# driskai/scenario_gym

Measured on AMD Instinct MI355X. Metric: entity-steps/sec (batched rollout), higher is better.
Workload: dtype f64

## Files before the change

scenario_gym_amd/csrc/sgym_control.hpp:

```cpp
#pragma once

namespace sg {

struct CtlLds { double ctrl[9][64]; double seg[5][64]; };

template <bool FAST, bool RIDERS = false>
__device__ __forceinline__ void control_body_l(CtlLds &lds ,
                                               const unsigned qblock ,
                                               const Params &p, double timestep, int n_steps, int first, int k0,
                                               const double *actions , double *tab, int row0, int metrics)
{
    const int lane = threadIdx.x;
    const size_t q = (size_t)qblock * 64 + lane;
    const int ent_raw = p.ctl_ent[q];
    const bool active = ent_raw >= 0;
    const uint32_t ent = active ? (uint32_t)ent_raw : 0u;
    const uint32_t r = ent / (uint32_t)p.EP;
    const LanePtr st(p.stat + (size_t)(ent >> 6) * (ST_COUNT * 64), (ent & 63) * 8u);
    const LanePtr dy(p.dyn + (size_t)(ent >> 6) * ((size_t)p.FROWS * 64), (ent & 63) * 8u);
    const int64_t meta = fld<int64_t>(st, ST_META);
    const int kind = active ? (int)(meta & 0xff) : SG_KIND_NONE;
    const double min_t = fld(st, ST_MIN_T), bl = fld(st, ST_BL);
    const bool is_ego = active && (int)(ent - r * (uint32_t)p.EP) == p.sstat[r].ego;
#pragma unroll
    for (int c = 0; c < 9; ++c) lds.ctrl[c][lane] = fld(st, ST_CTRL + c);
    const size_t NP = (size_t)p.n_ctl_pad;
    double *cst = p.ctl_state + q;

    double pose[6], t, prev_t;
    double m_avg, m_max, m_t;
    bool present;
    CtrlState cs;
    if (first) {
        const sg_scenario_state &sd = p.sdyn[r];
        t = sd.t;
        prev_t = sd.prev_t;
        m_avg = sd.ego_avg_speed; m_max = sd.ego_max_speed; m_t = sd.avg_t;
        present = fld<uint64_t>(dy, SG_F_PRESENT) != 0;
#pragma unroll
        for (int c = 0; c < 6; ++c) pose[c] = fld(dy, SG_F_POSE + c);
        cs.speed = fld(dy, SG_F_CTRL + 0); cs.e_lon_prev = fld(dy, SG_F_CTRL + 1);
        cs.e_lat_prev = fld(dy, SG_F_CTRL + 2); cs.e_lon_int = fld(dy, SG_F_CTRL + 3);
    } else {
#pragma unroll
        for (int c = 0; c < 6; ++c) pose[c] = cst[(CS_POSE + c) * NP];
        present = cst[CS_PRESENT * NP] != 0.0;
        cs.speed = cst[(CS_CTRL + 0) * NP]; cs.e_lon_prev = cst[(CS_CTRL + 1) * NP];
        cs.e_lat_prev = cst[(CS_CTRL + 2) * NP]; cs.e_lon_int = cst[(CS_CTRL + 3) * NP];
        t = cst[CS_T * NP];
        prev_t = cst[CS_PREV_T * NP];
        m_avg = cst[(CS_METRIC + 0) * NP]; m_max = cst[(CS_METRIC + 1) * NP]; m_t = cst[(CS_METRIC + 2) * NP];
    }
    if (!active) present = false;

    Table T;
    {
        const double *kn = p.knots + fld<int64_t>(st, ST_KNOT_OFF) * 7;
        T.x = kn; T.xs = 7; T.y = kn + 1; T.ys = 7; T.cs = 1;
        T.n = active ? (int)(meta >> 32) : 0;
    }
    double seg_hi;
    int seg_cur;
    double sgr[5] = {0.0, 0.0, 0.0, 0.0, 0.0};
    auto seg_publish = [&](const Segment &S) {
        lds.seg[0][lane] = S.x_lo;
        lds.seg[1][lane] = S.ylo[0]; lds.seg[2][lane] = S.ylo[1];
        lds.seg[3][lane] = S.sl[0]; lds.seg[4][lane] = S.sl[1];
        if (FAST) { sgr[0] = S.x_lo; sgr[1] = S.ylo[0]; sgr[2] = S.ylo[1]; sgr[3] = S.sl[0]; sgr[4] = S.sl[1]; }
        seg_hi = S.x_hi;
        seg_cur = S.cur;
    };
    {
        Segment S;
        S.cur = seg_locate(T, t);
        seg_load(T, S);
        seg_publish(S);
    }
    double *out = tab + (q * (size_t)(p.tab_steps + 1) + (size_t)row0) * CT_W;
    double *out1 = out + (size_t)p.n_ctl_pad * ((size_t)(p.tab_steps + 1) * CT_W);
    double *out2 = out1 + (size_t)p.n_ctl_pad * ((size_t)(p.tab_steps + 1) * CT_W);
    const bool replay_lane = RIDERS && (kind == SG_KIND_REPLAY || kind == SG_KIND_AGENT_REPLAY);
    const double max_t = fld(st, ST_MAX_T);
    const bool is_static = (int)(meta >> 32) == 1;
    Table TR{};
    Segment SR{};
    if (RIDERS) {
        TR = lane_table(p, replay_lane ? kind : SG_KIND_NONE, p.sstat[r], (int)(ent - r * (uint32_t)p.EP), st);
        if (!replay_lane) TR.n = 0;
        SR.cur = seg_locate(TR, t);
        seg_load(TR, SR);
    }
    sg_loads_done();
    const bool fast_kind = FAST && !p.ctl_general && sg_all(!active || (kind == SG_KIND_AGENT_PID && bl > 0.0 && bl < 0x1p400));
    const RecipDiv rd_l(active ? bl : 1.0), rd_10(10.0);
    double cpr[9];
#pragma unroll
    for (int c = 0; c < 9; ++c) cpr[c] = FAST ? fld(st, ST_CTRL + c) : 0.0;
    sg_loads_done();

    for (int k = 0; k < n_steps; ++k) {
        const double *Kp = SG_TRIG;
        if (!FAST) asm volatile("" : "+s"(Kp));
        ConstTbl K = (ConstTbl)Kp;
        const double next_t = t + timestep;
        const double state_dt = t - prev_t;
        const double dt = next_t - t;
        if (FAST && fast_kind && sg_all(!active || (present && !(next_t > seg_hi) && __builtin_fabs(pose[3]) < 1.0e5))) {
            const double dq = next_t - sgr[0];
            const double tx = sgr[3] * dq + sgr[1], ty = sgr[4] * dq + sgr[2];
            double sin_h, cos_h;
            sg_sincos_core(pose[3], sin_h, cos_h, K);
            const double e0 = tx - pose[0], e1 = ty - pose[1];
            const double e_lon = cos_h * e0 + sin_h * e1;
            const double e_lat = -sin_h * e0 + cos_h * e1;
            const double speed0 = cs.speed;
            const double g_mid = 1.0 - rd_10.div(0.9 * (speed0 - 5.0));
            const double gain = (speed0 > 5.0 && speed0 <= 15) ? g_mid : (speed0 > 15 ? 0.1 : 1.0);
            const RecipDiv rd(state_dt);
            const double d_lat = e_lat - cs.e_lat_prev, d_lon = e_lon - cs.e_lon_prev;
            const double e_lat_D = rd.div(d_lat);
            const double kp = cpr[SG_C_STEER_KP] * gain, kd = cpr[SG_C_STEER_KD] * gain;
            double steer = kp * e_lat + kd * e_lat_D;
            const double e_lon_D = rd.div(d_lon);
            const double e_lon_I = cs.e_lon_int + e_lon * state_dt;
            double accel = cpr[SG_C_ACCEL_KP] * e_lon + cpr[SG_C_ACCEL_KD] * e_lon_D + cpr[SG_C_ACCEL_KI] * e_lon_I;
            accel = __builtin_fabs(e_lon) > 0.1 ? accel : 0.0;
            const double max_steer = cpr[SG_C_MAX_STEER], max_accel = cpr[SG_C_MAX_ACCEL];
            const double max_speed = cpr[SG_C_MAX_SPEED], allow_rev = cpr[SG_C_ALLOW_REVERSE];
            accel = __builtin_fmin(__builtin_fmax(accel, -max_accel), max_accel);
            steer = __builtin_fmin(__builtin_fmax(steer, -max_steer), max_steer);
            const double dxs = speed0 * cos_h, dys = speed0 * sin_h;
            double tan_s = sg_tan_poly(steer, K);
            const bool steep = !(__builtin_fabs(steer) < 0.67434);
            if (sg_any(steep & active)) {
                double s2, c2;
                sg_sincos_core(steer, s2, c2, K);
                tan_s = steep ? s2 / c2 : tan_s;
            }
            const double hnum = speed0 * tan_s;
            const double dh = hnum == 0.0 ? hnum : rd_l.div(hnum);
            const double nx = pose[0] + dxs * dt, ny = pose[1] + dys * dt, nh = pose[3] + dh * dt;
            double nspeed = speed0 + accel * dt;
            nspeed = allow_rev == 0.0 ? __builtin_fmax(0.0, nspeed) : nspeed;
            nspeed = max_speed == max_speed ? __builtin_fmin(max_speed, nspeed) : nspeed;
            bool ok = rd.safe(d_lat) & rd.safe(d_lon) & (__builtin_fabs(steer) < 1.0e5) & (rd_l.safe(hnum) | (hnum == 0.0));
            double n_avg = m_avg, n_max = m_max, n_mt = m_t;
            if (metrics) {
                const RecipDiv rdt(dt), rnt(next_t);
                const double ax = nx - pose[0], ay = ny - pose[1];
                const double az = pose[2] - pose[2];
                const double speed = sg_norm3(rdt.div(ax), rdt.div(ay), 0.0);
                const double w = rnt.div(m_t);
                n_avg = m_avg + (1.0 - w) * (speed - m_avg);
                n_max = __builtin_fmax(speed, m_max);
                n_mt = next_t;
                ok = ok & (!is_ego | (rdt.safe(ax) & rdt.safe(ay) & rnt.safe(m_t) & (dt > 0.0) & (az == 0.0)));
            }
            if (sg_all(!active || ok)) {
                cs.e_lat_prev = e_lat; cs.e_lon_prev = e_lon; cs.e_lon_int = e_lon_I; cs.speed = nspeed;
                pose[0] = nx; pose[1] = ny; pose[3] = nh;
                if (is_ego) { m_avg = n_avg; m_max = n_max; m_t = n_mt; }
                prev_t = t;
                t = next_t;
                *reinterpret_cast<double4 *>(out + (size_t)k * CT_W) = make_double4(pose[0], pose[1], pose[3], cs.speed);
                *reinterpret_cast<double4 *>(out1 + (size_t)k * CT_W) = make_double4(cs.e_lon_prev, cs.e_lat_prev, cs.e_lon_int, 0.0);
                if (is_ego && metrics) *reinterpret_cast<double4 *>(out2 + (size_t)k * CT_W) = make_double4(m_avg, m_max, m_t, 0.0);
                continue;
            }
        }
        double act_a = 0.0, act_s = 0.0;
        if (kind == SG_KIND_AGENT_VEHICLE && actions) {
            const double *a = actions + ((size_t)(k0 + k) * p.R + r) * 2;
            act_a = a[0];
            act_s = a[1];
        }
        if (next_t > seg_hi) {
            Segment S;
            S.x_hi = seg_hi;
            S.cur = seg_cur;
            seg_advance(T, S, next_t);
            seg_publish(S);
            sg_loads_done();
        }
        double np_[6];
        const double dq = next_t - lds.seg[0][lane];
        np_[0] = lds.seg[3][lane] * dq + lds.seg[1][lane];
        np_[1] = lds.seg[4][lane] * dq + lds.seg[2][lane];
        bool npres = false;
        if (RIDERS && replay_lane) {
            if (next_t > SR.x_hi) { seg_advance(TR, SR, next_t); sg_loads_done(); }
            const double dqr = next_t - SR.x_lo;
#pragma unroll
            for (int c = 0; c < 6; ++c) np_[c] = SR.sl[c] * dqr + SR.ylo[c];
            npres = kind == SG_KIND_REPLAY ? (p.persist || is_static || (next_t >= min_t && next_t <= max_t))
                                           : (present || min_t >= t);
        } else if (present) {
            npres = true;
            const double tx = np_[0], ty = np_[1];
#pragma unroll
            for (int c = 0; c < 6; ++c) np_[c] = pose[c];
            double sin_h, cos_h;
            sg_sincos(pose[3], sin_h, cos_h, K);
            auto cp = [&](int q) -> double { return lds.ctrl[q][lane]; };
            if (kind == SG_KIND_AGENT_PID)
                pid_step(cs, cp, bl, state_dt, dt, tx, ty, sin_h, cos_h, np_, K);
            else
                vehicle_step(cs, cp, bl, dt, act_a, act_s, sin_h, cos_h, np_, K);
        } else if (active && min_t >= t) {
            npres = true;
            Segment S;
            S.cur = seg_cur;
            seg_load(T, S);
            sg_loads_done();
            const double dqs = next_t - S.x_lo;
#pragma unroll
            for (int c = 0; c < 6; ++c) np_[c] = S.sl[c] * dqs + S.ylo[c];
        }
        if (is_ego && npres && metrics) {
            double prev[6];
            if (!present) {
                own_position_extrap(T.x, T.n, t, prev);
                sg_loads_done();
            } else {
#pragma unroll
                for (int c = 0; c < 6; ++c) prev[c] = pose[c];
            }
            const double v0 = (np_[0] - prev[0]) / dt, v1 = (np_[1] - prev[1]) / dt, v2 = (np_[2] - prev[2]) / dt;
            const double speed = sg_norm3(v0, v1, v2);
            const double w = m_t / next_t;
            m_avg += (1.0 - w) * (speed - m_avg);
            m_t = next_t;
            m_max = __builtin_fmax(speed, m_max);
        }
        present = npres;
        if (npres) {
#pragma unroll
            for (int c = 0; c < 6; ++c) pose[c] = np_[c];
        }
        prev_t = t;
        t = next_t;
        *reinterpret_cast<double4 *>(out + (size_t)k * CT_W) = make_double4(pose[0], pose[1], pose[3], cs.speed);
        *reinterpret_cast<double4 *>(out1 + (size_t)k * CT_W) = make_double4(cs.e_lon_prev, cs.e_lat_prev, cs.e_lon_int, 0.0);
        if (is_ego && metrics) *reinterpret_cast<double4 *>(out2 + (size_t)k * CT_W) = make_double4(m_avg, m_max, m_t, 0.0);
        if (RIDERS) *reinterpret_cast<double4 *>(out2 + (size_t)k * CT_W) = make_double4(pose[2], pose[4], pose[5], present ? 1.0 : 0.0);
    }
#pragma unroll
    for (int c = 0; c < 6; ++c) cst[(CS_POSE + c) * NP] = pose[c];
    cst[CS_PRESENT * NP] = present ? 1.0 : 0.0;
    cst[(CS_CTRL + 0) * NP] = cs.speed; cst[(CS_CTRL + 1) * NP] = cs.e_lon_prev;
    cst[(CS_CTRL + 2) * NP] = cs.e_lat_prev; cst[(CS_CTRL + 3) * NP] = cs.e_lon_int;
    cst[CS_T * NP] = t;
    cst[CS_PREV_T * NP] = prev_t;
    cst[(CS_METRIC + 0) * NP] = m_avg; cst[(CS_METRIC + 1) * NP] = m_max; cst[(CS_METRIC + 2) * NP] = m_t;
}

template <bool FAST, bool RIDERS = false>
__device__ __forceinline__ void control_body(const Params &p, double timestep, int n_steps, int first, int k0,
                                             const double *actions , double *tab, int row0, int metrics)
{
    __shared__ CtlLds lds;
    control_body_l<FAST, RIDERS>(lds, blockIdx.x, p, timestep, n_steps, first, k0, actions, tab, row0, metrics);
}

#ifdef SG_UNIT_CTL
static __global__ __launch_bounds__(64, SG_CTL_WAVES) void control_kernel(Params p, double timestep, int n_steps, int first, int k0,
                                                     const double *actions , double *tab, int row0, int metrics)
{
    control_body<false>(p, timestep, n_steps, first, k0, actions, tab, row0, metrics);
}
#endif
#ifdef SG_UNIT_CTL
static __global__ __launch_bounds__(64, 2) void control_kernel_riders(Params p, double timestep, int n_steps, int first, int k0,
                                                               const double *actions , double *tab, int row0, int metrics)
{
    control_body<false, true>(p, timestep, n_steps, first, k0, actions, tab, row0, 0);
}
#endif
#ifdef SG_UNIT_CTL
static __global__ __launch_bounds__(64, 1) void control_kernel_fast(Params p, double timestep, int n_steps, int first, int k0,
                                                             const double *actions , double *tab, int row0, int metrics)
{
#ifdef SG_CTL_SETPRIO
    __builtin_amdgcn_s_setprio(3);
#endif
    control_body<true>(p, timestep, n_steps, first, k0, actions, tab, row0, metrics);
}
#endif

}
```

scenario_gym_amd/csrc/sgym_core.hpp:

```cpp
#pragma once

namespace sg {

enum {
    ST_BW = 0, ST_BL, ST_BCX, ST_BCY,
    ST_MIN_T, ST_MAX_T,
    ST_KNOT_OFF,
    ST_META,
    ST_ROUTE,
    ST_CTL,
    ST_CTRL,
    NCTRL_ROWS = 13,
    ST_COUNT = ST_CTRL + NCTRL_ROWS
};
constexpr uint32_t ROW = 512;

struct ScenStatic {
    double t0, length;
    int64_t grid_off;
    int32_t grid_n, ego;
};

struct RoadNet { double x0, y0, inv_cell; int32_t nx, ny; int64_t cell_base; };
struct RoadCand { int32_t poly; uint32_t edge_off; uint16_t n_edges; uint8_t ref_sel, ref_inside; };
// ... 48 lines not shown
    int ctl_general;
    int ped_serial;
    int quiet;
    int tab_steps;
    int noise_mode;
    double noise_std_lon, noise_std_lat;
    const double *noise_normals;
    long long noise_len;
    unsigned long long noise_seed;
    int ped_behaviour;
    int n_ped_models;
    const double *ped_models;
    const int32_t *model_of;
#ifdef SG_PHASE_TIMERS
    unsigned long long *phase_cycles;
#endif
};

enum { PM_BEHAVIOUR = 0, PM_SF = 1, PM_STD_LON = 13, PM_STD_LAT = 14, PM_W = 16 };
static_assert(sizeof(sg_social_force) == 12 * sizeof(double), "sg_social_force is twelve doubles");

enum { CT_X = 0, CT_Y, CT_H, CT_SPEED, CT_W = 4, CT_ELON = 0, CT_ELAT, CT_EINT, CT_MAVG = 0, CT_MMAX, CT_MT, CT_PLANES = 3 };
enum { CS_POSE = 0, CS_PRESENT = 6, CS_CTRL = 7, CS_T = 11, CS_PREV_T = 12, CS_METRIC = 13, CS_COUNT = 16 };

#define SG_GLOBAL __attribute__((address_space(1)))
struct LanePtr {
    SG_GLOBAL char *a[3];
    __device__ __forceinline__ LanePtr(const double *blk, uint32_t voff)
    {
        a[0] = (SG_GLOBAL char *)(reinterpret_cast<char *>(const_cast<double *>(blk)) + voff);
        a[1] = a[0] + 8 * ROW;
        a[2] = a[0] + 16 * ROW;
        asm("" : "+v"(a[1]), "+v"(a[2]));
    }
};
template <typename T = double>
__device__ __forceinline__ T fld(const LanePtr &lp, int f)
{
    const int b = f < 24 ? f >> 3 : 2;
    return *reinterpret_cast<SG_GLOBAL const T *>(lp.a[b] + (f - 8 * b) * (int)ROW);
}
template <typename T>
__device__ __forceinline__ void stf(const LanePtr &lp, int f, T v)
{
    const int b = f < 24 ? f >> 3 : 2;
    *reinterpret_cast<SG_GLOBAL T *>(lp.a[b] + (f - 8 * b) * (int)ROW) = v;
}

__device__ __forceinline__ double sg_norm3(double a, double b, double c)
{
    return __builtin_sqrt(__builtin_fma(c, c, __builtin_fma(b, b, a * a)));
}
__device__ __forceinline__ double sg_norm2(double a, double b)
{
    return __builtin_sqrt(__builtin_fma(b, b, a * a));
}

__device__ __noinline__ double2 sg_sincos_slow(double x)
{
    return make_double2(sin(x), cos(x));
}

static __constant__ double SG_TRIG[48] = {
    6.36619772367581382433e-01,
    1.57079632673412561417e+00,
    6.07710050630396597660e-11,
    2.02226624879595063154e-21,
    -1.66666666666666324348e-01, 8.33333333332248946124e-03, -1.98412698298579493134e-04,
    2.75573137070700676789e-06, -2.50507602534068634195e-08, 1.58969099521155010221e-10,
    4.16666666666666019037e-02, -1.38888888888741095749e-03, 2.48015872894767294178e-05,
    -2.75573143513906633035e-07, 2.08757232129817482790e-09, -1.13596475577881948265e-11,
    3.33333333333334091986e-01, 1.33333333333201242699e-01, 5.39682539762260521377e-02,
    2.18694882948595424599e-02, 8.86323982359930005737e-03, 3.59207910759131235356e-03,
    1.45620945432529025516e-03, 5.88041240820264096874e-04, 2.46463134818469906812e-04,
    7.81794442939557092300e-05, 7.14072491382608190305e-05, -1.85586374855275456654e-05,
    2.59073051863633712884e-05, 0.0, 0.0, 0.0,
    3.33333333333329318027e-01, -1.99999999998764832476e-01, 1.42857142725034663711e-01, -1.11111104054623557880e-01,
    9.09088713343650656196e-02, -7.69187620504482999495e-02, 6.66107313738753120669e-02, -5.83357013379057348645e-02,
    4.97687799461593236017e-02, -3.65315727442169155270e-02, 1.62858201153657823623e-02, 0.0, 0.0, 0.0, 0.0, 0.0,
};

typedef const __attribute__((address_space(4))) double *ConstTbl;

__device__ __forceinline__ void sg_sincos_core(double x, double &s, double &c, ConstTbl K);

__device__ __forceinline__ void sg_sincos(double x, double &s, double &c, ConstTbl K = (ConstTbl)SG_TRIG)
{
    if (!(__builtin_fabs(x) < 1.0e5)) {
        double2 sc = sg_sincos_slow(x);
        s = sc.x;
        c = sc.y;
        return;
    }
    sg_sincos_core(x, s, c, K);
}

__device__ __forceinline__ void sg_sincos_core(double x, double &s, double &c, ConstTbl K)
{
    double fn = __builtin_rint(x * K[0]);
    int n = (int)fn;
    double t = x - fn * K[1];
    double w = fn * K[2];
    double r = t - w;
    w = fn * K[3] - ((t - r) - w);
    double y0 = r - w;
    double y1 = (r - y0) - w;
    double z = y0 * y0;
    double v = z * y0;
    double rs = K[5] + z * (K[6] + z * (K[7] + z * (K[8] + z * K[9])));
    double ks = y0 - ((z * (0.5 * y1 - v * rs) - y1) - v * K[4]);
    double rc = z * (K[10] + z * (K[11] + z * (K[12] + z * (K[13] + z * (K[14] + z * K[15])))));
    double ay = __builtin_fabs(y0);
    uint64_t qb = ((uint64_t)__double_as_longlong(ay) - ((uint64_t)0x00200000 << 32)) & 0xFFFFFFFF00000000ULL;
    double qx = ay > 0.78125 ? 0.28125 : __longlong_as_double((long long)qb);
    qx = ay < 0.3 ? 0.0 : qx;
    double hz = 0.5 * z - qx;
    double a = 1.0 - qx;
    double kc = a - (hz - (z * rc - y0 * y1));
    double ss = (n & 1) ? kc : ks;
    double cc = (n & 1) ? ks : kc;
    s = (n & 2) ? -ss : ss;
    c = ((n + 1) & 2) ? -cc : cc;
}

__device__ __forceinline__ double sg_tan_poly(double x, ConstTbl K)
{
    ConstTbl T = K + 16;
    double z = x * x;
    double w = z * z;
    double r = T[1] + w * (T[3] + w * (T[5] + w * (T[7] + w * (T[9] + w * T[11]))));
    double v = z * (T[2] + w * (T[4] + w * (T[6] + w * (T[8] + w * (T[10] + w * T[12])))));
    double s = z * x;
    r = z * (s * (r + v));
    r = r + T[0] * s;
    return x + r;
}

__device__ __forceinline__ double sg_tan(double x, ConstTbl K)
{
    if (!(__builtin_fabs(x) < 0.67434)) {
        double s, c;
        sg_sincos(x, s, c, K);
        return s / c;
    }
    return sg_tan_poly(x, K);
}

#define SG_TRIG32_ERR 4.0e-6f
__device__ __forceinline__ void sg_sincos_f32(double h, float &s, float &c)
{
    if (!(__builtin_fabs(h) < 1.0e5)) {
        double2 sc = sg_sincos_slow(h);
        s = (float)sc.x;
        c = (float)sc.y;
        return;
    }
    const double rev = h * 1.59154943091895345554e-01;
    const float f = (float)(rev - __builtin_rint(rev));
    s = __builtin_amdgcn_sinf(f);
    c = __builtin_amdgcn_cosf(f);
}

__device__ __forceinline__ double sg_pred(double x)
{
    long long b = __double_as_longlong(x);
    if (x > 0.0) return __longlong_as_double(b - 1);
    if (x < 0.0) return __longlong_as_double(b + 1);
    return -4.9406564584124654e-324;
}

__device__ __forceinline__ bool sg_any(bool p) { return __builtin_amdgcn_ballot_w64(p) != 0; }
__device__ __forceinline__ bool sg_all(bool p) { return __builtin_amdgcn_ballot_w64(!p) == 0; }

__device__ __forceinline__ double shfl_d(double v, int src) { return __shfl(v, src, 64); }

__device__ __forceinline__ void sg_loads_done() { __builtin_amdgcn_s_waitcnt(0x0F70); }
__device__ __forceinline__ void sg_lgkm_done() { __builtin_amdgcn_s_waitcnt(0xC07F); }

struct RecipDiv {
    double b, r;
    bool ok;
    __device__ __forceinline__ explicit RecipDiv(double den) : b(den)
    {
        double ab = __builtin_fabs(den);
        ok = ab > 0x1p-500 && ab < 0x1p500;
        double r0 = __builtin_amdgcn_rcp(den);
        double e0 = __builtin_fma(-den, r0, 1.0);
        double r1 = __builtin_fma(r0, e0, r0);
        double e1 = __builtin_fma(-den, r1, 1.0);
        r = __builtin_fma(r1, e1, r1);
    }
    __device__ __forceinline__ bool safe(double a) const
    {
        uint32_t e = ((uint32_t)__double2hiint(a) >> 20) & 0x7ffu;
        return ok & (((e - 64u) < 1920u) | (__double_as_longlong(a) == 0));
    }
    __device__ __forceinline__ double div(double a) const
    {
        double q0 = a * r;
        double e = __builtin_fma(-b, q0, a);
        return __builtin_fma(e, r, q0);
    }
};

struct Table {
    const double *x;
    const double *y;
    int n;
    int xs, ys, cs;
    __device__ __forceinline__ double X(int i) const { return x[(size_t)i * xs]; }
    __device__ __forceinline__ double Y(int i, int c) const { return y[(size_t)i * ys + (size_t)c * cs]; }
};

struct Segment {
    double x_lo, x_hi;
    double ylo[6], sl[6];
    int cur;
};

__device__ __forceinline__ void seg_load(const Table &T, Segment &S)
{
    const int n = T.n, cur = S.cur;
    if (n <= 0) {
        S.x_lo = 0.0;
        S.x_hi = __builtin_inf();
#pragma unroll
        for (int c = 0; c < 6; ++c) { S.ylo[c] = 0.0; S.sl[c] = 0.0; }
        return;
    }
    if (cur == 0 || cur >= n || n == 1) {
        int row = cur == 0 ? 0 : n - 1;
        double x0 = T.X(row);
        S.x_lo = x0;
        S.x_hi = (cur == 0 && n > 1) ? sg_pred(x0) : __builtin_inf();
#pragma unroll
        for (int c = 0; c < 6; ++c) { S.ylo[c] = T.Y(row, c); S.sl[c] = 0.0; }
        return;
    }
    double x_lo = T.X(cur - 1), x_hi = T.X(cur);
    S.x_lo = x_lo;
    S.x_hi = x_hi;
    double dx = x_hi - x_lo;
#pragma unroll
    for (int c = 0; c < 6; ++c) {
        double a = T.Y(cur - 1, c), b = T.Y(cur, c);
        S.ylo[c] = a;
        S.sl[c] = (b - a) / dx;
    }
}

__device__ __forceinline__ int seg_locate(const Table &T, double t)
{
    const int n = T.n;
    if (n <= 1) return 0;
    if (t < T.X(0)) return 0;
    if (t > T.X(n - 1)) return n;
    int lo = 0, hi = n;
    while (lo < hi) {
        int mid = (lo + hi) >> 1;
        if (T.X(mid) < t) lo = mid + 1; else hi = mid;
    }
    return lo < 1 ? 1 : (lo > n - 1 ? n - 1 : lo);
}

__device__ __forceinline__ void seg_advance(const Table &T, Segment &S, double t)
{
    if (t > S.x_hi) {
        int cur = S.cur == 0 ? 1 : S.cur;
        while (cur <= T.n - 1 && T.X(cur) < t) ++cur;
        S.cur = cur;
        seg_load(T, S);
    }
}

__device__ __forceinline__ void own_position_extrap(const double *kn, int n, double t, double (&out)[6])
{
    if (n == 1) {
        double x_lo = kn[0];
// ... 104 lines not shown
```

scenario_gym_amd/csrc/sgym_queue.hpp:

```cpp
#pragma once

namespace sg {

enum { Q_TICKET = 0, Q_HEAD = 1, Q_ERR = 2, Q_ITEMS_DONE = 3, Q_CTL_CLAIMED = 4, Q_STATE_WORDS = 8 };
constexpr int Q_SEATS = 1 << 14;
enum { Q_ERR_CTL_WAIT = 1, Q_ERR_BLOCK_WAIT = 2, Q_ERR_RING_WAIT = 3 };
constexpr int Q_MAX_CHUNKS = 255;
constexpr int Q_PROG_STRIDE = 32;

struct TabQueue {
    unsigned *state;
    unsigned *ctl_prog;
    unsigned *blk_prog;
    unsigned *chunk_cnt;
    unsigned *seats;
    long long defer_ticks;
    double *tab;
    size_t buf_doubles;
    const double *actions;
    unsigned *trace;
    unsigned long long *times;
    long long timeout_ticks;
    int n_chunks, n_buf, nblk, n_ctl_waves;
    int nap;
// ... 26 lines not shown
        }
    }
}

__device__ __forceinline__ void q_acquire()
{
    __builtin_amdgcn_fence(__ATOMIC_ACQUIRE, "agent");
    asm volatile("s_dcache_inv\n\ts_waitcnt lgkmcnt(0)" ::: "memory");
}

__device__ __forceinline__ void q_release()
{
    asm volatile("s_waitcnt vmcnt(0)" ::: "memory");
    __builtin_amdgcn_fence(__ATOMIC_RELEASE, "agent");
    asm volatile("s_waitcnt vmcnt(0)" ::: "memory");
}

template <int G>
__device__ __forceinline__ void q_handoff_writethrough(const Params &p, unsigned b, int lane)
{
    asm volatile("s_waitcnt vmcnt(0)" ::: "memory");
    typedef SG_GLOBAL unsigned long long gu64;
    constexpr int FR = SG_F_COLL + 1;
    gu64 *rows = (gu64 *)(p.dyn + (size_t)b * ((size_t)FR * 64)) + lane;
    unsigned long long v[FR];
#pragma unroll
    for (int f = 0; f < FR; ++f) v[f] = __hip_atomic_load(rows + f * 64, __ATOMIC_RELAXED, __HIP_MEMORY_SCOPE_AGENT);
#pragma unroll
    for (int f = 0; f < FR; ++f) __hip_atomic_store(rows + f * 64, v[f], __ATOMIC_RELAXED, __HIP_MEMORY_SCOPE_AGENT);
    static_assert(sizeof(sg_scenario_state) % 8 == 0, "scenario records are copied in 8-byte words");
    constexpr int SW = (int)(sizeof(sg_scenario_state) / 8);
    const int gl = (int)b * 64 + lane, r = gl / G, slot = gl & (G - 1);
    if (r < p.R) {
        gu64 *sd = (gu64 *)(p.sdyn + r);
        for (int w = slot; w < SW; w += G) {
            const unsigned long long v = __hip_atomic_load(sd + w, __ATOMIC_RELAXED, __HIP_MEMORY_SCOPE_AGENT);
            __hip_atomic_store(sd + w, v, __ATOMIC_RELAXED, __HIP_MEMORY_SCOPE_AGENT);
        }
    }
    asm volatile("s_waitcnt vmcnt(0)" ::: "memory");
}

template <int G, unsigned F>
__device__ __forceinline__ void tabq_body(const Params &p, double timestep, int force, const TabQueue &tq)
{
    constexpr bool RSS = (F & V_RSS) != 0;
    using Tile = typename Variant<G, 1, F>::Lds;
    static_assert(sizeof(Tile) >= sizeof(CtlLds), "the pre-pass role lays its LDS over the tile");
    __shared__ Tile lds;
    __shared__ typename std::conditional<RSS, RssQueue, char>::type rssq_lds;
    const int lane = threadIdx.x;
    unsigned ticket = ~0u;
    {
        const unsigned hw = (unsigned)__builtin_amdgcn_s_getreg((4 << 0) | (0 << 6) | (31 << 11));
        const unsigned xcc = (unsigned)__builtin_amdgcn_s_getreg((20 << 0) | (0 << 6) | (3 << 11));
        const unsigned seat = ((xcc & 15u) << 10) | (((hw >> 13) & 7u) << 7) | (((hw >> 12) & 1u) << 6) | (((hw >> 8) & 15u) << 2) | ((hw >> 4) & 3u);
        unsigned rank = 0;
        if (lane == 0) {
            atomicAdd(tq.state + Q_TICKET, 1u);
            rank = atomicAdd(tq.seats + seat, 1u);
        }
        rank = (unsigned)__builtin_amdgcn_readfirstlane((int)rank);
        bool claim = rank == 0 && q_peek(tq.state + Q_CTL_CLAIMED) < (unsigned)tq.n_ctl_waves;
        if (rank != 0) {
            const long long t0 = wall_clock64();
            while (q_peek(tq.state + Q_CTL_CLAIMED) < (unsigned)tq.n_ctl_waves) {
                if (wall_clock64() - t0 > tq.defer_ticks) { claim = true; break; }
                __builtin_amdgcn_s_sleep(8);
            }
        }
        if (claim) {
            unsigned idx = 0;
            if (lane == 0) idx = atomicAdd(tq.state + Q_CTL_CLAIMED, 1u);
            idx = (unsigned)__builtin_amdgcn_readfirstlane((int)idx);
            if (idx < (unsigned)tq.n_ctl_waves) ticket = idx;
        }
    }

    if (ticket < (unsigned)tq.n_ctl_waves) {
        __builtin_amdgcn_s_setprio(3);
        CtlLds &cl = *reinterpret_cast<CtlLds *>(&lds);
        for (int c = 0; c < tq.n_chunks; ++c) {
            if (c >= tq.n_buf && !q_wait_ge(tq.chunk_cnt + (c - tq.n_buf), (unsigned)tq.nblk, tq, Q_ERR_RING_WAIT)) break;
            control_body_l<true>(cl, ticket, p, timestep, tq.k0[c + 1] - tq.k0[c], c == 0, tq.k0[c], tq.actions,
                                 tq.tab + (size_t)(c % tq.n_buf) * tq.buf_doubles, 0, RSS ? 0 : 1);
            q_release();
            if (tq.times && lane == 0) tq.times[(size_t)tq.n_chunks * tq.nblk * 4 + (size_t)ticket * tq.n_chunks + c] = wall_clock64();
            if (lane == 0) __hip_atomic_store(tq.ctl_prog + ticket * Q_PROG_STRIDE, (unsigned)(c + 1), __ATOMIC_RELAXED, __HIP_MEMORY_SCOPE_AGENT);
        }
        __builtin_amdgcn_s_setprio(0);
        if (q_peek(tq.state + Q_ERR) != 0) return;
    }

    const unsigned n_items = (unsigned)tq.n_chunks * (unsigned)tq.nblk;
    unsigned done_b = ~0u, done_c = 0;
    for (;;) {
        unsigned item = 0;
        if (lane == 0) {
            if (done_b != ~0u) {
                __hip_atomic_store(tq.blk_prog + done_b, done_c + 1, __ATOMIC_RELAXED, __HIP_MEMORY_SCOPE_AGENT);
                if (tq.n_buf < tq.n_chunks) atomicAdd(tq.chunk_cnt + done_c, 1u);
                atomicAdd(tq.state + Q_ITEMS_DONE, 1u);
            }
            item = atomicAdd(tq.state + Q_HEAD, 1u);
        }
        item = (unsigned)__builtin_amdgcn_readfirstlane((int)item);
        done_b = ~0u;
        if (item >= n_items) break;
        const unsigned c = item / (unsigned)tq.nblk, b = item - c * (unsigned)tq.nblk;
        auto trace = [&](unsigned stage) {
            if (tq.trace && lane == 0) __hip_atomic_store(tq.trace + b, (c << 8) | stage, __ATOMIC_RELAXED, __HIP_MEMORY_SCOPE_AGENT);
        };
        trace(1);
        auto stamp = [&](int k) {
            if (tq.times && lane == 0) tq.times[(size_t)item * 4 + k] = wall_clock64();
        };
        stamp(0);
        if (tq.lag_prio) __builtin_amdgcn_s_setprio(0);
        const bool behind = c != 0 && q_peek(tq.blk_prog + b) < c;
        bool ok = c == 0 || q_wait_ge(tq.blk_prog + b, c, tq, Q_ERR_BLOCK_WAIT);
        {
            const LanePtr st(p.stat + (size_t)b * (ST_COUNT * 64), (uint32_t)lane * 8u);
            const int64_t cq = fld<int64_t>(st, ST_CTL);
            uint64_t m = __ballot(cq >= 0);
            while (m && ok) {
                const int l = __builtin_ctzll(m);
                m &= m - 1;
                const unsigned w = (unsigned)__builtin_amdgcn_readlane((int)(uint32_t)cq, l) >> 6;
                ok = q_wait_ge(tq.ctl_prog + w * Q_PROG_STRIDE, c + 1, tq, Q_ERR_CTL_WAIT);
            }
        }
        if (!ok) break;
        if (tq.lag_prio && behind) {
            if (tq.lag_prio == 1) __builtin_amdgcn_s_setprio(1);
            else __builtin_amdgcn_s_setprio(2);
        }
        trace(2);
        q_acquire();
        trace(3);
        stamp(1);
        const double *tab = tq.tab + (size_t)(c % (unsigned)tq.n_buf) * tq.buf_doubles;
        const int gl = (int)b * 64 + lane, r_raw = gl / G;
        const bool in_range = r_raw < p.R;
        const int r = in_range ? r_raw : p.R - 1;
        const int ev_before = p.ev_cap > 0 ? min(p.sdyn[r].n_events, p.ev_cap) : 0;
        rollout_body_l<G, 1, F>(lds, p, timestep, tq.k0[c + 1] - tq.k0[c], 0, force, nullptr, tab, SliceArgs{}, b);
        trace(4);
        stamp(2);
        if (RSS) {
            asm volatile("s_waitcnt vmcnt(0)" ::: "memory");
            rss_lines_block(p, (RssQueueLds)&rssq_lds, (size_t)b);
        }
        if (!RSS && p.ev_cap > 0) {
            asm volatile("s_waitcnt vmcnt(0)" ::: "memory");
            const int ev_after = in_range ? min(p.sdyn[r].n_events, p.ev_cap) : 0;
            if (ev_after > ev_before) {
                int64_t ectl;
                const bool from_tab = ego_table_column(p, r, ectl);
                for (int i = ev_before + (gl & (G - 1)); i < ev_after; i += G) event_take_table_pose(p, r, i, tab, from_tab, ectl);
            }
        }
        trace(5);
        if (RSS) {
            asm volatile("s_waitcnt vmcnt(0)" ::: "memory");
            typedef SG_GLOBAL int gi32;
            typedef SG_GLOBAL unsigned long long gu64;
            const size_t idx = (size_t)b * 64 + lane;
            gi32 *sw = (gi32 *)(p.rss_state + idx), *cw = (gi32 *)(p.rss_code + idx);
// ... 51 lines not shown
```

Measured before the change: 148.0 billion.

## Reorder fast PID step for ILP, carry reciprocal across steps, use LDS body

Reorders the fast-path control step so the steering chain, metrics and longitudinal work are interleaved, shortening the dependency chain per step. The reciprocal of the previous dt is carried across iterations, so a fresh RecipDiv of state_dt is no longer computed each step. The fast kernel now calls the LDS-based body with metrics as a compile-time-like branch, and the tan polynomial is interleaved explicitly. Numerics could shift slightly if the carried reciprocal differs from recomputing it.

```diff
diff --git a/scenario_gym_amd/csrc/sgym_control.hpp b/scenario_gym_amd/csrc/sgym_control.hpp
--- a/scenario_gym_amd/csrc/sgym_control.hpp
+++ b/scenario_gym_amd/csrc/sgym_control.hpp
@@ -97,6 +97,7 @@
 #pragma unroll
     for (int c = 0; c < 9; ++c) cpr[c] = FAST ? fld(st, ST_CTRL + c) : 0.0;
     sg_loads_done();
+    RecipDiv rdc(FAST ? t - prev_t : 1.0);
 
     for (int k = 0; k < n_steps; ++k) {
         const double *Kp = SG_TRIG;
@@ -106,32 +107,53 @@
         const double state_dt = t - prev_t;
         const double dt = next_t - t;
         if (FAST && fast_kind && sg_all(!active || (present && !(next_t > seg_hi) && __builtin_fabs(pose[3]) < 1.0e5))) {
+            RecipDiv rd = rdc;
+            rd.b = state_dt;
+            const RecipDiv rdt(dt);
             const double dq = next_t - sgr[0];
             const double tx = sgr[3] * dq + sgr[1], ty = sgr[4] * dq + sgr[2];
+            const double speed0 = cs.speed;
+            const double g_mid = 1.0 - rd_10.div(0.9 * (speed0 - 5.0));
+            const double gain = (speed0 > 5.0 && speed0 <= 15) ? g_mid : (speed0 > 15 ? 0.1 : 1.0);
+            const double kp = cpr[SG_C_STEER_KP] * gain, kd = cpr[SG_C_STEER_KD] * gain;
+            const double max_steer = cpr[SG_C_MAX_STEER], max_accel = cpr[SG_C_MAX_ACCEL];
+            const double max_speed = cpr[SG_C_MAX_SPEED], allow_rev = cpr[SG_C_ALLOW_REVERSE];
+            const RecipDiv rnt(metrics ? next_t : 1.0);
+            const double w = rnt.div(m_t);
             double sin_h, cos_h;
             sg_sincos_core(pose[3], sin_h, cos_h, K);
             const double e0 = tx - pose[0], e1 = ty - pose[1];
+            const double e_lat = -sin_h * e0 + cos_h * e1;
+            const double d_lat = e_lat - cs.e_lat_prev;
+            const double e_lat_D = rd.div(d_lat);
+            double steer = kp * e_lat + kd * e_lat_D;
+            steer = __builtin_fmin(__builtin_fmax(steer, -max_steer), max_steer);
+            double tan_s = sg_tan_poly(steer, K);
+            const bool steep = !(__builtin_fabs(steer) < 0.67434);
+            const double dxs = speed0 * cos_h, dys = speed0 * sin_h;
+            const double nx = pose[0] + dxs * dt, ny = pose[1] + dys * dt;
+            double n_avg = m_avg, n_max = m_max, n_mt = m_t;
+            bool ok = rd.safe(d_lat) & (__builtin_fabs(steer) < 1.0e5);
+            if (metrics) {
+                const double ax = nx - pose[0], ay = ny - pose[1];
+                const double az = pose[2] - pose[2];
+                const double speed = sg_norm3(rdt.div(ax), rdt.div(ay), 0.0);
+                n_avg = m_avg + (1.0 - w) * (speed - m_avg);
+                n_max = __builtin_fmax(speed, m_max);
+                n_mt = next_t;
+                ok = ok & (!is_ego | (rdt.safe(ax) & rdt.safe(ay) & rnt.safe(m_t) & (dt > 0.0) & (az == 0.0)));
+            }
             const double e_lon = cos_h * e0 + sin_h * e1;
-            const double e_lat = -sin_h * e0 + cos_h * e1;
-            const double speed0 = cs.speed;
-            const double g_mid = 1.0 - rd_10.div(0.9 * (speed0 - 5.0));
-            const double gain = (speed0 > 5.0 && speed0 <= 15) ? g_mid : (speed0 > 15 ? 0.1 : 1.0);
-            const RecipDiv rd(state_dt);
-            const double d_lat = e_lat - cs.e_lat_prev, d_lon = e_lon - cs.e_lon_prev;
-            const double e_lat_D = rd.div(d_lat);
-            const double kp = cpr[SG_C_STEER_KP] * gain, kd = cpr[SG_C_STEER_KD] * gain;
-            double steer = kp * e_lat + kd * e_lat_D;
+            const double d_lon = e_lon - cs.e_lon_prev;
             const double e_lon_D = rd.div(d_lon);
             const double e_lon_I = cs.e_lon_int + e_lon * state_dt;
             double accel = cpr[SG_C_ACCEL_KP] * e_lon + cpr[SG_C_ACCEL_KD] * e_lon_D + cpr[SG_C_ACCEL_KI] * e_lon_I;
             accel = __builtin_fabs(e_lon) > 0.1 ? accel : 0.0;
-            const double max_steer = cpr[SG_C_MAX_STEER], max_accel = cpr[SG_C_MAX_ACCEL];
-            const double max_speed = cpr[SG_C_MAX_SPEED], allow_rev = cpr[SG_C_ALLOW_REVERSE];
             accel = __builtin_fmin(__builtin_fmax(accel, -max_accel), max_accel);
-            steer = __builtin_fmin(__builtin_fmax(steer, -max_steer), max_steer);
-            const double dxs = speed0 * cos_h, dys = speed0 * sin_h;
-            double tan_s = sg_tan_poly(steer, K);
-            const bool steep = !(__builtin_fabs(steer) < 0.67434);
+            double nspeed = speed0 + accel * dt;
+            nspeed = allow_rev == 0.0 ? __builtin_fmax(0.0, nspeed) : nspeed;
+            nspeed = max_speed == max_speed ? __builtin_fmin(max_speed, nspeed) : nspeed;
+            ok = ok & rd.safe(d_lon);
             if (sg_any(steep & active)) {
                 double s2, c2;
                 sg_sincos_core(steer, s2, c2, K);
@@ -139,24 +161,10 @@
             }
             const double hnum = speed0 * tan_s;
             const double dh = hnum == 0.0 ? hnum : rd_l.div(hnum);
-            const double nx = pose[0] + dxs * dt, ny = pose[1] + dys * dt, nh = pose[3] + dh * dt;
-            double nspeed = speed0 + accel * dt;
-            nspeed = allow_rev == 0.0 ? __builtin_fmax(0.0, nspeed) : nspeed;
-            nspeed = max_speed == max_speed ? __builtin_fmin(max_speed, nspeed) : nspeed;
-            bool ok = rd.safe(d_lat) & rd.safe(d_lon) & (__builtin_fabs(steer) < 1.0e5) & (rd_l.safe(hnum) | (hnum == 0.0));
-            double n_avg = m_avg, n_max = m_max, n_mt = m_t;
-            if (metrics) {
-                const RecipDiv rdt(dt), rnt(next_t);
-                const double ax = nx - pose[0], ay = ny - pose[1];
-                const double az = pose[2] - pose[2];
-                const double speed = sg_norm3(rdt.div(ax), rdt.div(ay), 0.0);
-                const double w = rnt.div(m_t);
-                n_avg = m_avg + (1.0 - w) * (speed - m_avg);
-                n_max = __builtin_fmax(speed, m_max);
-                n_mt = next_t;
-                ok = ok & (!is_ego | (rdt.safe(ax) & rdt.safe(ay) & rnt.safe(m_t) & (dt > 0.0) & (az == 0.0)));
-            }
+            const double nh = pose[3] + dh * dt;
+            ok = ok & (rd_l.safe(hnum) | (hnum == 0.0));
             if (sg_all(!active || ok)) {
+                rdc = rdt;
                 cs.e_lat_prev = e_lat; cs.e_lon_prev = e_lon; cs.e_lon_int = e_lon_I; cs.speed = nspeed;
                 pose[0] = nx; pose[1] = ny; pose[3] = nh;
                 if (is_ego) { m_avg = n_avg; m_max = n_max; m_t = n_mt; }
@@ -237,6 +245,7 @@
 #pragma unroll
             for (int c = 0; c < 6; ++c) pose[c] = np_[c];
         }
+        if (FAST) rdc = RecipDiv(dt);
         prev_t = t;
         t = next_t;
         *reinterpret_cast<double4 *>(out + (size_t)k * CT_W) = make_double4(pose[0], pose[1], pose[3], cs.speed);
@@ -283,7 +292,9 @@
 #ifdef SG_CTL_SETPRIO
     __builtin_amdgcn_s_setprio(3);
 #endif
-    control_body<true>(p, timestep, n_steps, first, k0, actions, tab, row0, metrics);
+    __shared__ CtlLds lds;
+    if (metrics) control_body_l<true>(lds, blockIdx.x, p, timestep, n_steps, first, k0, actions, tab, row0, 1);
+    else control_body_l<true>(lds, blockIdx.x, p, timestep, n_steps, first, k0, actions, tab, row0, 0);
 }
 #endif
 
diff --git a/scenario_gym_amd/csrc/sgym_core.hpp b/scenario_gym_amd/csrc/sgym_core.hpp
--- a/scenario_gym_amd/csrc/sgym_core.hpp
+++ b/scenario_gym_amd/csrc/sgym_core.hpp
@@ -200,9 +200,18 @@
     ConstTbl T = K + 16;
     double z = x * x;
     double w = z * z;
-    double r = T[1] + w * (T[3] + w * (T[5] + w * (T[7] + w * (T[9] + w * T[11]))));
-    double v = z * (T[2] + w * (T[4] + w * (T[6] + w * (T[8] + w * (T[10] + w * T[12])))));
     double s = z * x;
+    double r = w * T[11], v = w * T[12];
+    r = T[9] + r;  v = T[10] + v;
+    r = w * r;     v = w * v;
+    r = T[7] + r;  v = T[8] + v;
+    r = w * r;     v = w * v;
+    r = T[5] + r;  v = T[6] + v;
+    r = w * r;     v = w * v;
+    r = T[3] + r;  v = T[4] + v;
+    r = w * r;     v = w * v;
+    r = T[1] + r;  v = T[2] + v;
+    v = z * v;
     r = z * (s * (r + v));
     r = r + T[0] * s;
     return x + r;
```

Result: no change. 148.3 billion (median of 3 runs) (+0.1%).

## Restructure fast PID control step into tight inner loop with register-held constants

Applied to the files above, without the earlier changes.

The fast control path becomes an inner loop that stays in the fast path across steps instead of re-entering the outer loop each time. The trig polynomial constants are loaded into registers once per iteration, the steep-steer branch is made branchless, and the state_dt reciprocal is carried from the previous step's dt reciprocal. Metrics are made a compile-time template parameter, and register pinning plus a scheduling barrier are used to shape instruction order. This removes repeated constant loads, a divergent branch and redundant reciprocal computations, at the cost of higher register pressure and always computing the steer sincos.

```diff
diff --git a/scenario_gym_amd/csrc/sgym_control.hpp b/scenario_gym_amd/csrc/sgym_control.hpp
--- a/scenario_gym_amd/csrc/sgym_control.hpp
+++ b/scenario_gym_amd/csrc/sgym_control.hpp
@@ -4,12 +4,14 @@
 
 struct CtlLds { double ctrl[9][64]; double seg[5][64]; };
 
-template <bool FAST, bool RIDERS = false>
+template <bool FAST, bool RIDERS = false, int MET = -1>
 __device__ __forceinline__ void control_body_l(CtlLds &lds ,
                                                const unsigned qblock ,
                                                const Params &p, double timestep, int n_steps, int first, int k0,
-                                               const double *actions , double *tab, int row0, int metrics)
-{
+                                               const double *actions , double *tab, int row0, int metrics_arg)
+{
+    static_assert(!FAST || MET >= 0, "the fast step takes `metrics` at compile time");
+    const bool metrics = MET < 0 ? metrics_arg != 0 : MET != 0;
     const int lane = threadIdx.x;
     const size_t q = (size_t)qblock * 64 + lane;
     const int ent_raw = p.ctl_ent[q];
@@ -91,83 +93,101 @@
         seg_load(TR, SR);
     }
     sg_loads_done();
-    const bool fast_kind = FAST && !p.ctl_general && sg_all(!active || (kind == SG_KIND_AGENT_PID && bl > 0.0 && bl < 0x1p400));
+    const bool fast_kind = FAST && !p.ctl_general && sg_all(!active || (kind == SG_KIND_AGENT_PID && bl > 0x1p-400 && bl < 0x1p400));
     const RecipDiv rd_l(active ? bl : 1.0), rd_10(10.0);
     double cpr[9];
 #pragma unroll
     for (int c = 0; c < 9; ++c) cpr[c] = FAST ? fld(st, ST_CTRL + c) : 0.0;
     sg_loads_done();
 
+    RecipDiv rd_c(FAST ? t - prev_t : 1.0);
+    const double *Kp = SG_TRIG;
+
     for (int k = 0; k < n_steps; ++k) {
-        const double *Kp = SG_TRIG;
-        if (!FAST) asm volatile("" : "+s"(Kp));
+        asm volatile("" : "+s"(Kp));
         ConstTbl K = (ConstTbl)Kp;
-        const double next_t = t + timestep;
-        const double state_dt = t - prev_t;
-        const double dt = next_t - t;
-        if (FAST && fast_kind && sg_all(!active || (present && !(next_t > seg_hi) && __builtin_fabs(pose[3]) < 1.0e5))) {
+        double next_t = t + timestep;
+        double dt = next_t - t;
+        bool finished = false;
+        if (FAST && fast_kind) for (;;) {
+            if (!sg_all(!active | (present & !(next_t > seg_hi) & (__builtin_fabs(pose[3]) < 1.0e5)))) break;
+            const TrigRegs KR(K);
+            __builtin_amdgcn_sched_barrier(0);
+            const RecipDiv rd = rd_c;
+            const double sdt = rd.b;
+            RecipDiv rdt(dt), rnt(metrics ? next_t : 1.0);
             const double dq = next_t - sgr[0];
             const double tx = sgr[3] * dq + sgr[1], ty = sgr[4] * dq + sgr[2];
-            double sin_h, cos_h;
-            sg_sincos_core(pose[3], sin_h, cos_h, K);
-            const double e0 = tx - pose[0], e1 = ty - pose[1];
-            const double e_lon = cos_h * e0 + sin_h * e1;
-            const double e_lat = -sin_h * e0 + cos_h * e1;
+            double e0 = tx - pose[0], e1 = ty - pose[1];
             const double speed0 = cs.speed;
             const double g_mid = 1.0 - rd_10.div(0.9 * (speed0 - 5.0));
             const double gain = (speed0 > 5.0 && speed0 <= 15) ? g_mid : (speed0 > 15 ? 0.1 : 1.0);
-            const RecipDiv rd(state_dt);
+            double kp = cpr[SG_C_STEER_KP] * gain, kd = cpr[SG_C_STEER_KD] * gain;
+            sg_pin(rdt.r); sg_pin(e0); sg_pin(e1); sg_pin(kp); sg_pin(kd);
+            if (metrics) sg_pin(rnt.r);
+            sg_pin(pose[3]);
+            double sin_h, cos_h;
+            sg_sincos_core(pose[3], sin_h, cos_h, KR);
+            const double e_lon = cos_h * e0 + sin_h * e1;
+            const double e_lat = -sin_h * e0 + cos_h * e1;
             const double d_lat = e_lat - cs.e_lat_prev, d_lon = e_lon - cs.e_lon_prev;
             const double e_lat_D = rd.div(d_lat);
-            const double kp = cpr[SG_C_STEER_KP] * gain, kd = cpr[SG_C_STEER_KD] * gain;
             double steer = kp * e_lat + kd * e_lat_D;
             const double e_lon_D = rd.div(d_lon);
-            const double e_lon_I = cs.e_lon_int + e_lon * state_dt;
+            double e_lon_I = cs.e_lon_int + e_lon * sdt;
             double accel = cpr[SG_C_ACCEL_KP] * e_lon + cpr[SG_C_ACCEL_KD] * e_lon_D + cpr[SG_C_ACCEL_KI] * e_lon_I;
             accel = __builtin_fabs(e_lon) > 0.1 ? accel : 0.0;
             const double max_steer = cpr[SG_C_MAX_STEER], max_accel = cpr[SG_C_MAX_ACCEL];
+            sg_pin(cpr[SG_C_MAX_SPEED]); sg_pin(cpr[SG_C_ALLOW_REVERSE]);
             const double max_speed = cpr[SG_C_MAX_SPEED], allow_rev = cpr[SG_C_ALLOW_REVERSE];
             accel = __builtin_fmin(__builtin_fmax(accel, -max_accel), max_accel);
             steer = __builtin_fmin(__builtin_fmax(steer, -max_steer), max_steer);
             const double dxs = speed0 * cos_h, dys = speed0 * sin_h;
-            double tan_s = sg_tan_poly(steer, K);
+            const double tan_p = sg_tan_poly(steer, KR);
             const bool steep = !(__builtin_fabs(steer) < 0.67434);
-            if (sg_any(steep & active)) {
-                double s2, c2;
-                sg_sincos_core(steer, s2, c2, K);
-                tan_s = steep ? s2 / c2 : tan_s;
-            }
+            double s2, c2;
+            sg_sincos_core(steer, s2, c2, KR);
+            const double tan_s = steep ? s2 / c2 : tan_p;
             const double hnum = speed0 * tan_s;
             const double dh = hnum == 0.0 ? hnum : rd_l.div(hnum);
-            const double nx = pose[0] + dxs * dt, ny = pose[1] + dys * dt, nh = pose[3] + dh * dt;
+            double nx = pose[0] + dxs * dt, ny = pose[1] + dys * dt, nh = pose[3] + dh * dt;
             double nspeed = speed0 + accel * dt;
             nspeed = allow_rev == 0.0 ? __builtin_fmax(0.0, nspeed) : nspeed;
             nspeed = max_speed == max_speed ? __builtin_fmin(max_speed, nspeed) : nspeed;
-            bool ok = rd.safe(d_lat) & rd.safe(d_lon) & (__builtin_fabs(steer) < 1.0e5) & (rd_l.safe(hnum) | (hnum == 0.0));
-            double n_avg = m_avg, n_max = m_max, n_mt = m_t;
+            bool ok = rd.safe(d_lat) & rd.safe(d_lon) & (__builtin_fabs(steer) < 1.0e5) & (RecipDiv::safe_num(hnum) | (hnum == 0.0));
+            double n_avg = m_avg, n_max = m_max;
             if (metrics) {
-                const RecipDiv rdt(dt), rnt(next_t);
                 const double ax = nx - pose[0], ay = ny - pose[1];
                 const double az = pose[2] - pose[2];
                 const double speed = sg_norm3(rdt.div(ax), rdt.div(ay), 0.0);
                 const double w = rnt.div(m_t);
                 n_avg = m_avg + (1.0 - w) * (speed - m_avg);
                 n_max = __builtin_fmax(speed, m_max);
-                n_mt = next_t;
-                ok = ok & (!is_ego | (rdt.safe(ax) & rdt.safe(ay) & rnt.safe(m_t) & (dt > 0.0) & (az == 0.0)));
+                const bool m_ok = rdt.safe(ax) & rdt.safe(ay) & rnt.safe(m_t) & (dt > 0.0) & (az == 0.0);
+                ok = ok & !(is_ego & !m_ok);
+                sg_pin(n_avg); sg_pin(n_max);
             }
-            if (sg_all(!active || ok)) {
+            sg_pin(nx); sg_pin(ny); sg_pin(nh); sg_pin(nspeed); sg_pin(e_lon_I);
+            if (!sg_all(!active || ok)) break;
+            {
                 cs.e_lat_prev = e_lat; cs.e_lon_prev = e_lon; cs.e_lon_int = e_lon_I; cs.speed = nspeed;
                 pose[0] = nx; pose[1] = ny; pose[3] = nh;
-                if (is_ego) { m_avg = n_avg; m_max = n_max; m_t = n_mt; }
+                if (metrics) { m_avg = is_ego ? n_avg : m_avg; m_max = is_ego ? n_max : m_max; m_t = is_ego ? next_t : m_t; }
                 prev_t = t;
                 t = next_t;
+                rd_c = rdt;
                 *reinterpret_cast<double4 *>(out + (size_t)k * CT_W) = make_double4(pose[0], pose[1], pose[3], cs.speed);
                 *reinterpret_cast<double4 *>(out1 + (size_t)k * CT_W) = make_double4(cs.e_lon_prev, cs.e_lat_prev, cs.e_lon_int, 0.0);
                 if (is_ego && metrics) *reinterpret_cast<double4 *>(out2 + (size_t)k * CT_W) = make_double4(m_avg, m_max, m_t, 0.0);
-                continue;
             }
-        }
+            if (++k >= n_steps) { finished = true; break; }
+            asm volatile("" : "+s"(Kp));
+            K = (ConstTbl)Kp;
+            next_t = t + timestep;
+            dt = next_t - t;
+        }
+        if (finished) break;
+        const double state_dt = t - prev_t;
         double act_a = 0.0, act_s = 0.0;
         if (kind == SG_KIND_AGENT_VEHICLE && actions) {
             const double *a = actions + ((size_t)(k0 + k) * p.R + r) * 2;
@@ -243,6 +263,7 @@
         *reinterpret_cast<double4 *>(out1 + (size_t)k * CT_W) = make_double4(cs.e_lon_prev, cs.e_lat_prev, cs.e_lon_int, 0.0);
         if (is_ego && metrics) *reinterpret_cast<double4 *>(out2 + (size_t)k * CT_W) = make_double4(m_avg, m_max, m_t, 0.0);
         if (RIDERS) *reinterpret_cast<double4 *>(out2 + (size_t)k * CT_W) = make_double4(pose[2], pose[4], pose[5], present ? 1.0 : 0.0);
+        if (FAST) rd_c = RecipDiv(t - prev_t);
     }
 #pragma unroll
     for (int c = 0; c < 6; ++c) cst[(CS_POSE + c) * NP] = pose[c];
@@ -259,7 +280,12 @@
                                              const double *actions , double *tab, int row0, int metrics)
 {
     __shared__ CtlLds lds;
-    control_body_l<FAST, RIDERS>(lds, blockIdx.x, p, timestep, n_steps, first, k0, actions, tab, row0, metrics);
+    if constexpr (!FAST)
+        control_body_l<false, RIDERS>(lds, blockIdx.x, p, timestep, n_steps, first, k0, actions, tab, row0, metrics);
+    else if (metrics)
+        control_body_l<FAST, RIDERS, 1>(lds, blockIdx.x, p, timestep, n_steps, first, k0, actions, tab, row0, 1);
+    else
+        control_body_l<FAST, RIDERS, 0>(lds, blockIdx.x, p, timestep, n_steps, first, k0, actions, tab, row0, 0);
 }
 
 #ifdef SG_UNIT_CTL
diff --git a/scenario_gym_amd/csrc/sgym_core.hpp b/scenario_gym_amd/csrc/sgym_core.hpp
--- a/scenario_gym_amd/csrc/sgym_core.hpp
+++ b/scenario_gym_amd/csrc/sgym_core.hpp
@@ -154,7 +154,18 @@
 
 typedef const __attribute__((address_space(4))) double *ConstTbl;
 
-__device__ __forceinline__ void sg_sincos_core(double x, double &s, double &c, ConstTbl K);
+template <typename KT>
+__device__ __forceinline__ void sg_sincos_core(double x, double &s, double &c, KT K);
+
+struct TrigRegs {
+    double v[29];
+    __device__ __forceinline__ explicit TrigRegs(ConstTbl K)
+    {
+#pragma unroll
+        for (int i = 0; i < 29; ++i) v[i] = K[i];
+    }
+    __device__ __forceinline__ double operator[](int i) const { return v[i]; }
+};
 
 __device__ __forceinline__ void sg_sincos(double x, double &s, double &c, ConstTbl K = (ConstTbl)SG_TRIG)
 {
@@ -167,7 +178,8 @@
     sg_sincos_core(x, s, c, K);
 }
 
-__device__ __forceinline__ void sg_sincos_core(double x, double &s, double &c, ConstTbl K)
+template <typename KT>
+__device__ __forceinline__ void sg_sincos_core(double x, double &s, double &c, KT K)
 {
     double fn = __builtin_rint(x * K[0]);
     int n = (int)fn;
@@ -195,16 +207,17 @@
     c = ((n + 1) & 2) ? -cc : cc;
 }
 
-__device__ __forceinline__ double sg_tan_poly(double x, ConstTbl K)
-{
-    ConstTbl T = K + 16;
+template <typename KT>
+__device__ __forceinline__ double sg_tan_poly(double x, KT K)
+{
+    constexpr int T = 16;
     double z = x * x;
     double w = z * z;
-    double r = T[1] + w * (T[3] + w * (T[5] + w * (T[7] + w * (T[9] + w * T[11]))));
-    double v = z * (T[2] + w * (T[4] + w * (T[6] + w * (T[8] + w * (T[10] + w * T[12])))));
+    double r = K[T + 1] + w * (K[T + 3] + w * (K[T + 5] + w * (K[T + 7] + w * (K[T + 9] + w * K[T + 11]))));
+    double v = z * (K[T + 2] + w * (K[T + 4] + w * (K[T + 6] + w * (K[T + 8] + w * (K[T + 10] + w * K[T + 12])))));
     double s = z * x;
     r = z * (s * (r + v));
-    r = r + T[0] * s;
+    r = r + K[T + 0] * s;
     return x + r;
 }
 
@@ -248,6 +261,7 @@
 
 __device__ __forceinline__ void sg_loads_done() { __builtin_amdgcn_s_waitcnt(0x0F70); }
 __device__ __forceinline__ void sg_lgkm_done() { __builtin_amdgcn_s_waitcnt(0xC07F); }
+__device__ __forceinline__ void sg_pin(double &v) { asm volatile("" : "+v"(v)); }
 
 struct RecipDiv {
     double b, r;
@@ -262,10 +276,11 @@
         double e1 = __builtin_fma(-den, r1, 1.0);
         r = __builtin_fma(r1, e1, r1);
     }
-    __device__ __forceinline__ bool safe(double a) const
+    __device__ __forceinline__ bool safe(double a) const { return ok & safe_num(a); }
+    static __device__ __forceinline__ bool safe_num(double a)
     {
         uint32_t e = ((uint32_t)__double2hiint(a) >> 20) & 0x7ffu;
-        return ok & (((e - 64u) < 1920u) | (__double_as_longlong(a) == 0));
+        return ((e - 64u) < 1920u) | (__double_as_longlong(a) == 0);
     }
     __device__ __forceinline__ double div(double a) const
     {
diff --git a/scenario_gym_amd/csrc/sgym_queue.hpp b/scenario_gym_amd/csrc/sgym_queue.hpp
--- a/scenario_gym_amd/csrc/sgym_queue.hpp
+++ b/scenario_gym_amd/csrc/sgym_queue.hpp
@@ -132,8 +132,8 @@
         CtlLds &cl = *reinterpret_cast<CtlLds *>(&lds);
         for (int c = 0; c < tq.n_chunks; ++c) {
             if (c >= tq.n_buf && !q_wait_ge(tq.chunk_cnt + (c - tq.n_buf), (unsigned)tq.nblk, tq, Q_ERR_RING_WAIT)) break;
-            control_body_l<true>(cl, ticket, p, timestep, tq.k0[c + 1] - tq.k0[c], c == 0, tq.k0[c], tq.actions,
-                                 tq.tab + (size_t)(c % tq.n_buf) * tq.buf_doubles, 0, RSS ? 0 : 1);
+            control_body_l<true, false, RSS ? 0 : 1>(cl, ticket, p, timestep, tq.k0[c + 1] - tq.k0[c], c == 0, tq.k0[c], tq.actions,
+                                                     tq.tab + (size_t)(c % tq.n_buf) * tq.buf_doubles, 0, RSS ? 0 : 1);
             q_release();
             if (tq.times && lane == 0) tq.times[(size_t)tq.n_chunks * tq.nblk * 4 + (size_t)ticket * tq.n_chunks + c] = wall_clock64();
             if (lane == 0) __hip_atomic_store(tq.ctl_prog + ticket * Q_PROG_STRIDE, (unsigned)(c + 1), __ATOMIC_RELAXED, __HIP_MEMORY_SCOPE_AGENT);
```

Result: no change. 150.6 billion before, 149.5 billion after (-0.7%).
